# melspectrum007/audio-visual-speech-enhancement

Hardware: NVIDIA B200
Metric: audio-sec/sec (higher is better)
Workload: dtype f32

## Files before the change

audio-visual-speech-enhancement_b200/csrc/avse_fwd4_stages.cuh:

```cuda
#pragma once
#include "avse_common.h"
#include "avse_dft.cuh"
#include "avse_fwd_stages.cuh"

#if !defined(AVSE_DB_FAST_MINMAX)
#define AVSE_DB_FAST_MINMAX 0
#endif
#if !defined(AVSE_SCAN4_UNROLL)
#define AVSE_SCAN4_UNROLL 8
#endif

namespace avse {

constexpr int F4 = 4;
constexpr int CHUNK4 = 41;
constexpr int SCAN4_BINS = 8 * CHUNK4;
constexpr int FRAME4_F = N1 * ROW_F + 16;
constexpr int ZERO4_F = N1 * ROW_F;
#ifndef AVSE_SCAN4_BLK
#define AVSE_SCAN4_BLK 4
#endif
#ifndef AVSE_DB_BRANCHFREE_EXTRA
#define AVSE_DB_BRANCHFREE_EXTRA 1
#endif
constexpr int FLUSH4_F = 1284;
constexpr int WARP4_SMEM_F = F4 * FRAME4_F;
constexpr int RAW4 = 16 + 4 * (F4 - 1);
static_assert(FLUSH4_F + 48 <= FRAME4_F && (FLUSH4_F % 2) == 0, "flush area");

struct Lane4Const {
    float win[16];
    vec2 tw[16];
};

AVSE_HD void lane4_const_init(int lane, const float* s_win, const vec2* s_tw, Lane4Const& lc) {
#pragma unroll
    for (int j = 0; j < 16; ++j) { lc.win[j] = s_win[N2 * j + lane]; lc.tw[j] = s_tw[j * N2 + lane]; }
}

template <typename S, bool TILED>
AVSE_HD bool group4_interior(const FwdTileT<S>& tl, int& nz_shift) {
    nz_shift = 0;
    const int a = tl.t0 * HOP - HALF;
    if (!(tl.nz != nullptr && a >= 0 && (tl.t0 + 3) * HOP + HALF <= tl.vmin && tl.t0 + 3 < tl.T)) return false;
    if (TILED && tl.period_n > 0) {
        const int j = a + tl.phase_n;
        const int q = j / tl.period_n;
        if ((j + (F4 - 1) * HOP + NFFT - 1) / tl.period_n != q) return false;
        nz_shift = tl.phase_n - q * tl.period_n;
    }
    return true;
}

AVSE_HD void p4_column(cpx (&x)[16], const vec2 (&tw)[16], float* dst) {
    dft16(x);
    cstore(dst, x[0]);
#pragma unroll
    for (int k1 = 1; k1 < 16; ++k1) cstore(dst + k1 * ROW_F, cmul(x[k1], tw[k1].x, tw[k1].y));
}

template <typename S>
AVSE_HD void p4_load_raw(const FwdTileT<S>& tl, int nz_shift, int lane, float (&rs)[RAW4], float (&rn)[RAW4]) {
    const int o = tl.t0 * HOP - HALF + lane;
    const S* ps = tl.sp + o;
    const S* pn = tl.nz + (o + nz_shift);
#pragma unroll
    for (int j = 0; j < RAW4; ++j) { rs[j] = (float)ps[N2 * j]; rn[j] = (float)pn[N2 * j]; }
}

#if !defined(AVSE_F4_REFLECT_FAST)
#define AVSE_F4_REFLECT_FAST 1
#endif
AVSE_HD int reflect_index(int i, int L) {
    i = i < 0 ? -i : i;
    const int m = 2 * (L - 1) - i;
    return i < m ? i : m;
}

template <typename S, bool PAD>
AVSE_HD bool group4_reflect_only(const FwdTileT<S>& tl) {
    return tl.nz != nullptr && (PAD || tl.vmin >= tl.L) && tl.period_n == 0 && tl.L >= 4 * NFFT;
}

template <typename S, bool PAD>
AVSE_HD void p4_load_raw_reflect(const FwdTileT<S>& tl, int lane, float (&rs)[RAW4], float (&rn)[RAW4]) {
    const int o = tl.t0 * HOP - HALF + lane;
    if (!PAD || tl.vmin >= tl.L) {
#pragma unroll
        for (int j = 0; j < RAW4; ++j) { const int i = reflect_index(o + N2 * j, tl.L); rs[j] = (float)tl.sp[i]; rn[j] = (float)tl.nz[i]; }
    } else {
#pragma unroll
        for (int j = 0; j < RAW4; ++j) {
            const int i = reflect_index(o + N2 * j, tl.L);
            rs[j] = i < tl.valid_s ? (float)tl.sp[i] : 0.0f;
            rn[j] = i < tl.valid_n ? (float)tl.nz[i] : 0.0f;
        }
    }
}

template <typename S, bool PAD>
AVSE_HD void p4_load_tail_raw_reflect(const FwdTileT<S>& tl, int lane, float (&rs)[16], float (&rn)[16]) {
    const int o = (tl.t0 + (lane >> 3)) * HOP - HALF + 32 + (lane & 7);
    if (!PAD || tl.vmin >= tl.L) {
#pragma unroll
        for (int j = 0; j < 16; ++j) { const int i = reflect_index(o + N2 * j, tl.L); rs[j] = (float)tl.sp[i]; rn[j] = (float)tl.nz[i]; }
    } else {
#pragma unroll
        for (int j = 0; j < 16; ++j) {
            const int i = reflect_index(o + N2 * j, tl.L);
            rs[j] = i < tl.valid_s ? (float)tl.sp[i] : 0.0f;
            rn[j] = i < tl.valid_n ? (float)tl.nz[i] : 0.0f;
        }
    }
}

template <typename S>
AVSE_HD void stage4_store_pcm_guarded(const FwdTileT<S>& tl, int lane, const float (&rs)[RAW4], const float (&rn)[RAW4], const float (&ts)[16],
                                      const float (&tn)[16]) {
    if (tl.mixed_pcm == nullptr) return;
    const int i0 = tl.t0 * HOP + lane;
#pragma unroll
    for (int j = 8; j < 24; ++j) {
        const int i = i0 + N2 * (j - 8);
        if (i < tl.L) tl.mixed_pcm[i] = rs[j] + tl.factor * (rn[j] * tl.gain);
    }
    const int i1 = (tl.t0 + (lane >> 3)) * HOP + 32 + (lane & 7);
#pragma unroll
    for (int j = 0; j < 4; ++j) {
        const int i = i1 + N2 * j;
        if (i < tl.L) tl.mixed_pcm[i] = ts[8 + j] + tl.factor * (tn[8 + j] * tl.gain);
    }
}

#if !defined(AVSE_P1_ROLL)
#define AVSE_P1_ROLL 9
#endif
template <typename S>
AVSE_HD void stage4_pass1_main(const FwdTileT<S>& tl, int lane, float (&rs)[RAW4], float (&rn)[RAW4],
                               const Lane4Const& lc, float* frames) {
    const float gain = tl.gain;
#if AVSE_P1_ROLL == 9
#pragma unroll
    for (int j = 0; j < RAW4; ++j) rn[j] *= gain;
    if (tl.mixed_pcm != nullptr) {
        float* pm = tl.mixed_pcm + tl.t0 * HOP + lane;
#pragma unroll
        for (int j = 8; j < 24; ++j) pm[N2 * (j - 8)] = rs[j] + tl.factor * rn[j];
    }
#pragma unroll
    for (int f = 0; f < F4; ++f) {
        cpx x[16];
#pragma unroll
        for (int j = 0; j < 16; ++j) x[j] = cmake(rs[4 * f + j] * lc.win[j], rn[4 * f + j] * lc.win[j]);
        p4_column(x, lc.tw, frames + f * FRAME4_F + 2 * lane);
    }
#elif AVSE_P1_ROLL == 0
#pragma unroll
    for (int j = 0; j < 12; ++j) rn[j] *= gain;
#pragma unroll
    for (int f = 0; f < F4; ++f) {
#pragma unroll
        for (int j = 12; j < 16; ++j) rn[4 * f + j] *= gain;
        if (tl.mixed_pcm != nullptr) {
            float* pm = tl.mixed_pcm + (tl.t0 + f) * HOP + lane;
#pragma unroll
            for (int j = 0; j < 4; ++j) pm[N2 * j] = rs[4 * f + 8 + j] + tl.factor * rn[4 * f + 8 + j];
        }
        cpx x[16];
#pragma unroll
        for (int j = 0; j < 16; ++j) x[j] = cmake(rs[4 * f + j] * lc.win[j], rn[4 * f + j] * lc.win[j]);
        p4_column(x, lc.tw, frames + f * FRAME4_F + 2 * lane);
    }
#else
    constexpr int STEP = AVSE_P1_ROLL == 4 ? 1 : 2;
    constexpr int W = 16 + 4 * (STEP - 1);
#pragma unroll
    for (int j = 0; j < 12; ++j) rn[j] *= gain;
    float* pm = tl.mixed_pcm != nullptr ? tl.mixed_pcm + tl.t0 * HOP + lane : nullptr;
    float* dst = frames + 2 * lane;
#pragma unroll 1
    for (int it = 0; it < F4 / STEP; ++it) {
#pragma unroll
        for (int j = 12; j < W; ++j) rn[j] *= gain;
#pragma unroll
        for (int f = 0; f < STEP; ++f) {
            if (pm != nullptr) {
#pragma unroll
                for (int j = 0; j < 4; ++j) pm[N2 * j] = rs[4 * f + 8 + j] + tl.factor * rn[4 * f + 8 + j];
                pm += HOP;
            }
            cpx x[16];
#pragma unroll
            for (int j = 0; j < 16; ++j) x[j] = cmake(rs[4 * f + j] * lc.win[j], rn[4 * f + j] * lc.win[j]);
            p4_column(x, lc.tw, dst);
            dst += FRAME4_F;
        }
#pragma unroll
        for (int j = 0; j + 4 * STEP < RAW4; ++j) { rs[j] = rs[j + 4 * STEP]; rn[j] = rn[j + 4 * STEP]; }
    }
#endif
}

template <typename S>
AVSE_HD void p4_load_tail_raw(const FwdTileT<S>& tl, int nz_shift, int lane, float (&rs)[16], float (&rn)[16]) {
    const int f = lane >> 3, n2 = 32 + (lane & 7);
    const int o = (tl.t0 + f) * HOP - HALF + n2;
    const S* ps = tl.sp + o;
    const S* pn = tl.nz + (o + nz_shift);
#pragma unroll
    for (int j = 0; j < 16; ++j) { rs[j] = (float)ps[N2 * j]; rn[j] = (float)pn[N2 * j]; }
}

template <typename S>
AVSE_HD void stage4_pass1_tail_compute(const FwdTileT<S>& tl, int lane, const float (&rs)[16], float (&rn)[16], const float* s_win,
                                       const vec2* s_tw, float* frames) {
    const int f = lane >> 3, n2 = 32 + (lane & 7);
#pragma unroll
    for (int j = 0; j < 16; ++j) rn[j] *= tl.gain;
    vec2 tw[16];
#pragma unroll
    for (int k1 = 1; k1 < 16; ++k1) tw[k1] = s_tw[k1 * N2 + n2];
    tw[0].x = 1.0f; tw[0].y = 0.0f;
    if (tl.mixed_pcm != nullptr) {
        float* pm = tl.mixed_pcm + (tl.t0 + f) * HOP + n2;
#pragma unroll
        for (int j = 0; j < 4; ++j) pm[N2 * j] = rs[8 + j] + tl.factor * rn[8 + j];
    }
    cpx x[16];
#pragma unroll
    for (int j = 0; j < 16; ++j) { const float w = s_win[N2 * j + n2]; x[j] = cmake(rs[j] * w, rn[j] * w); }
    p4_column(x, tw, frames + f * FRAME4_F + 2 * n2);
}

template <typename S>
AVSE_HD void stage4_pass1_tail(const FwdTileT<S>& tl, int nz_shift, int lane, const float* s_win, const vec2* s_tw, float* frames) {
    float rs[16], rn[16];
    p4_load_tail_raw(tl, nz_shift, lane, rs, rn);
    stage4_pass1_tail_compute(tl, lane, rs, rn, s_win, s_tw, frames);
}

template <typename S>
AVSE_HD void stage4_pass1_unified(const FwdTileT<S>& tl, int lane, float (&rs)[RAW4], float (&rn)[RAW4], const float (&ts)[16], float (&tn)[16],
                                  const Lane4Const& lc, const float* s_win, const vec2* s_tw, float* frames) {
    const float gain = tl.gain;
    const int tf = lane >> 3, tn2 = 32 + (lane & 7);
#pragma unroll
    for (int j = 0; j < RAW4; ++j) rn[j] *= gain;
#pragma unroll
    for (int j = 0; j < 16; ++j) tn[j] *= gain;
    if (tl.mixed_pcm != nullptr) {
        float* pm = tl.mixed_pcm + tl.t0 * HOP + lane;
#pragma unroll
        for (int j = 8; j < 24; ++j) pm[N2 * (j - 8)] = rs[j] + tl.factor * rn[j];
        float* pt = tl.mixed_pcm + (tl.t0 + tf) * HOP + tn2;
#pragma unroll
        for (int j = 0; j < 4; ++j) pt[N2 * j] = ts[8 + j] + tl.factor * tn[8 + j];
    }
    vec2 tw[16];
    tw[0].x = 1.0f; tw[0].y = 0.0f;
#pragma unroll 1
    for (int round = 0; round < 5; ++round) {
        if (round == 0 || round == 4) {
            const int n2 = round == 0 ? lane : tn2;
#pragma unroll
            for (int k1 = 1; k1 < 16; ++k1) tw[k1] = s_tw[k1 * N2 + n2];
        }
        cpx x[16];
        float* dst;
        switch (round) {
        case 0:
#pragma unroll
            for (int j = 0; j < 16; ++j) x[j] = cmake(rs[j] * lc.win[j], rn[j] * lc.win[j]);
            dst = frames + 2 * lane;
            break;
        case 1:
#pragma unroll
            for (int j = 0; j < 16; ++j) x[j] = cmake(rs[4 + j] * lc.win[j], rn[4 + j] * lc.win[j]);
            dst = frames + FRAME4_F + 2 * lane;
            break;
        case 2:
#pragma unroll
            for (int j = 0; j < 16; ++j) x[j] = cmake(rs[8 + j] * lc.win[j], rn[8 + j] * lc.win[j]);
            dst = frames + 2 * FRAME4_F + 2 * lane;
            break;
        case 3:
#pragma unroll
            for (int j = 0; j < 16; ++j) x[j] = cmake(rs[12 + j] * lc.win[j], rn[12 + j] * lc.win[j]);
            dst = frames + 3 * FRAME4_F + 2 * lane;
            break;
        default:
#pragma unroll
            for (int j = 0; j < 16; ++j) { const float w = s_win[N2 * j + tn2]; x[j] = cmake(ts[j] * w, tn[j] * w); }
            dst = frames + tf * FRAME4_F + 2 * tn2;
            break;
        }
        p4_column(x, tw, dst);
    }
}

template <typename S, bool TILED>
AVSE_HD void stage4_pass1_edge(const FwdTileT<S>& tl, int lane, const float* s_win, const vec2* s_tw, float* frames) {
#pragma unroll 1
    for (int round = 0; round < 5; ++round) {
        const int f = round < 4 ? round : lane >> 3;
        const int n2 = round < 4 ? lane : 32 + (lane & 7);
        const int t_raw = tl.t0 + f;
        const int t = t_raw < tl.T ? t_raw : tl.T - 1;
        const int base = t * HOP - HALF + n2;
        float rs[16], rn[16];
#pragma unroll
        for (int j = 0; j < 16; ++j) {
            rs[j] = load_sample_edge(tl.sp, base + N2 * j, tl.L, tl.valid_s);
            rn[j] = tl.gain * load_sample_edge(tl.nz, base + N2 * j, tl.L, tl.valid_n, TILED ? tl.period_n : 0, TILED ? tl.phase_n : 0);
        }
        if (tl.mixed_pcm != nullptr && t_raw < tl.T) {
#pragma unroll
            for (int j = 0; j < 4; ++j) {
                const int i = t * HOP + N2 * j + n2;
                if (i < tl.L) tl.mixed_pcm[i] = rs[8 + j] + tl.factor * rn[8 + j];
            }
        }
        vec2 tw[16];
#pragma unroll
        for (int k1 = 1; k1 < 16; ++k1) tw[k1] = s_tw[k1 * N2 + n2];
        tw[0].x = 1.0f; tw[0].y = 0.0f;
        cpx x[16];
#pragma unroll
        for (int j = 0; j < 16; ++j) { const float w = s_win[N2 * j + n2]; x[j] = cmake(rs[j] * w, rn[j] * w); }
        p4_column(x, tw, frames + f * FRAME4_F + 2 * n2);
    }
}

AVSE_HD void p4_pass2_load(int lane, int r, const float* frames, cpx (&x)[40]) {
    const int f = 2 * r + (lane >> 4), k1 = lane & 15;
    const float* row = frames + f * FRAME4_F + k1 * ROW_F;
#pragma unroll
    for (int q = 0; q < 20; ++q) cload2(row + 4 * q, x[2 * q], x[2 * q + 1]);
}

AVSE_HD void p4_pass2_compute(int lane, int r, const float* frames, cpx (&x)[40]) {
    p4_pass2_load(lane, r, frames, x);
    dft40_inplace(x);
}

AVSE_HD void p4_pass2_store(int lane, int r, float* frames, const cpx (&x)[40]) {
    const int f = 2 * r + (lane >> 4), k1 = lane & 15;
    float* z = frames + f * FRAME4_F + 2 * k1;
#pragma unroll
    for (int c = 0; c < 5; ++c)
#pragma unroll
        for (int d = 0; d < 8; ++d) {
            const int idx = (8 * c + 5 * d) % 40;
            const int k2 = (16 * c + 25 * d) % 40;
            cstore(z + 2 * N1 * k2, x[idx]);
        }
}

AVSE_HD float fma_rn(float a, float b, float c) { return fmaf(a, b, c); }

AVSE_HD void scan4_bin(const float* za, const float* zc, const vec2* tab, int j, bool emit, float factor, float nfactor,
                       float*& esn, float*& em, cpx& Asn, cpx& Bsn, float& Am, float& Bm) {
    const cpx a = cload(za + 2 * j);
    const cpx c = cload(zc - 2 * j);
    const vec2 w = tab[j];
    if (emit) {
        cstore(esn, Asn);
        *em = Am;
        esn += 2;
        em -= 1;
        Asn = Bsn; Am = Bm;
        Bsn = cmake(0.0f, 0.0f); Bm = 0.0f;
    }
    const cpx s = cfma_pp(c, cmake(1.0f, -1.0f), a);
    const cpx n = cfma_pp(c, cmake(-1.0f, 1.0f), a);
    const float mr = fma_rn(factor, cim(n), cre(s));
    const float mi = fma_rn(nfactor, cre(n), cim(s));
    const float ms = fast_sqrt(fma_rn(cim(s), cim(s), cre(s) * cre(s)));
    const float mn = fast_sqrt(fma_rn(cim(n), cim(n), cre(n) * cre(n)));
    const float mm = fast_sqrt(fma_rn(mi, mi, mr * mr));
    const cpx msn = cmake(ms, mn);
    Asn = cfma_pp(msn, cmake(w.x, w.x), Asn);
    Bsn = cfma_pp(msn, cmake(w.y, w.y), Bsn);
    Am = fma_rn(w.x, mm, Am);
    Bm = fma_rn(w.y, mm, Bm);
}

AVSE_HD void stage4_scan(int lane, float factor, const vec2* s_w, unsigned mask_lo, unsigned mask_hi, float* frames) {
    const int f = lane >> 3, p = lane & 7;
    float* fr = frames + f * FRAME4_F;
    const float* za = fr + 2 * CHUNK4 * p;
    const float* zc = fr + 2 * (NFFT - CHUNK4 * p);
    const vec2* tab = s_w + CHUNK4 * p;
    float* esn = fr + 2 * CHUNK4 * p;
    float* em = fr + 2 * (NFFT - CHUNK4 * p) + 1;
    cpx Asn = cmake(0.0f, 0.0f), Bsn = cmake(0.0f, 0.0f);
    float Am = 0.0f, Bm = 0.0f;
    const float nfactor = -factor;
    unsigned mlo = mask_lo, mhi = mask_hi;
    static_assert(CHUNK4 == 41 && (40 % AVSE_SCAN4_BLK) == 0 && AVSE_SCAN4_BLK < 32, "blocks of AVSE_SCAN4_BLK bins + 1");
#pragma unroll 1
    for (int ib = 0; ib < 40; ib += AVSE_SCAN4_BLK) {
#pragma unroll
        for (int j = 0; j < AVSE_SCAN4_BLK; ++j) scan4_bin(za, zc, tab, j, ((mlo >> j) & 1u) != 0u, factor, nfactor, esn, em, Asn, Bsn, Am, Bm);
        za += 2 * AVSE_SCAN4_BLK; zc -= 2 * AVSE_SCAN4_BLK; tab += AVSE_SCAN4_BLK;
        mlo = (mlo >> AVSE_SCAN4_BLK) | (mhi << (32 - AVSE_SCAN4_BLK));
        mhi >>= AVSE_SCAN4_BLK;
    }
    scan4_bin(za, zc, tab, 0, (mlo & 1u) != 0u, factor, nfactor, esn, em, Asn, Bsn, Am, Bm);
    float* fl = fr + FLUSH4_F + 6 * p;
    cstore(fl + 0, Asn);
    cstore(fl + 2, Bsn);
    cstore(fl + 4, cmake(Am, Bm));
}

AVSE_HD void stage4_db(int lane, int q, float factor, const ivec4* s_loc, const float* frames, const FwdOut& out, int t0, int T,
                       float (&mx)[3], float* mn) {
    const int m = 32 * q + lane;
    if (m >= NMEL) return;
    const ivec4 loc = s_loc[m];
    float mel[3][F4];
#pragma unroll
    for (int f = 0; f < F4; ++f) {
        const float* fr = frames + f * FRAME4_F;
        const vec2 sn = *reinterpret_cast<const vec2*>(fr + (loc.x & 0xffff));
        mel[0][f] = sn.x; mel[1][f] = sn.y; mel[2][f] = fr[loc.x >> 16];
    }
#if AVSE_DB_BRANCHFREE_EXTRA
    {
#pragma unroll
        for (int f = 0; f < F4; ++f) {
            const float* fr = frames + f * FRAME4_F;
            const vec2 sn = *reinterpret_cast<const vec2*>(fr + (loc.y & 0xffff));
            mel[0][f] += sn.x; mel[1][f] += sn.y; mel[2][f] += fr[loc.y >> 16];
        }
    }
#else
    if ((loc.y & 0xffff) != ZERO4_F) {
#pragma unroll
        for (int f = 0; f < F4; ++f) {
            const float* fr = frames + f * FRAME4_F;
            const vec2 sn = *reinterpret_cast<const vec2*>(fr + (loc.y & 0xffff));
            mel[0][f] += sn.x; mel[1][f] += sn.y; mel[2][f] += fr[loc.y >> 16];
        }
    }
#endif
    if (loc.z >= 0) {
#pragma unroll
        for (int f = 0; f < F4; ++f) {
            const float* fr = frames + f * FRAME4_F;
            const vec2 sn = *reinterpret_cast<const vec2*>(fr + (loc.z & 0xffff));
            mel[0][f] += sn.x; mel[1][f] += sn.y; mel[2][f] += fr[loc.z >> 16];
        }
    }
    const int nvalid = T - t0 < F4 ? T - t0 : F4;
    int off;
    bool store = true;
    if (out.layout == 0) {
        const int sl = t0 / SPSS, tt = t0 - sl * SPSS;
        off = (sl * NMEL + m) * SPSS + tt;
        store = sl < out.n_slices;
    } else {
        off = m * out.ld_t + t0;
    }
#pragma unroll
    for (int sig = 0; sig < 3; ++sig) {
        const float scale = sig == 1 ? factor : 1.0f;
        float d[F4];
        float lm = neg_inf(), ln = -neg_inf();
#pragma unroll
        for (int f = 0; f < F4; ++f) d[f] = amp_to_db(mel[sig][f] * scale);
#if AVSE_DB_FAST_MINMAX
        if (nvalid == F4) {
            lm = fmaxf(fmaxf(d[0], d[1]), fmaxf(d[2], d[3]));
            ln = fminf(fminf(d[0], d[1]), fminf(d[2], d[3]));
        } else
#endif
        {
#pragma unroll
            for (int f = 0; f < F4; ++f) {
                const bool v = f < nvalid;
                lm = v ? fmaxf(lm, d[f]) : lm;
                ln = v ? fminf(ln, d[f]) : ln;
            }
        }
        mx[sig] = fmaxf(lm, mx[sig]);
        float* dst = out.dst[sig];
        mn[32 * sig + lane] = fminf(mn[32 * sig + lane], (dst != nullptr && store) ? ln : -neg_inf());
        if (dst != nullptr && store) {
            if (out.layout == 0) {
                vec4 o; o.x = d[0]; o.y = d[1]; o.z = d[2]; o.w = d[3];
                *reinterpret_cast<vec4*>(dst + off) = o;
            } else {
#pragma unroll
                for (int f = 0; f < F4; ++f)
                    if (f < nvalid) dst[off + f] = d[f];
            }
        }
    }
}

#if !defined(AVSE_DB_SPLIT_LAST)
#define AVSE_DB_SPLIT_LAST 1
#endif
AVSE_HD void stage4_db_last(int lane, float factor, const ivec4* s_loc, const float* frames, const FwdOut& out, int t0, int T,
                            float (&mx)[3], float* mn) {
    const int half = lane >> 4, m = 64 + (lane & 15), f0 = 2 * half;
    const ivec4 loc = s_loc[m];
    float mel[3][2];
#pragma unroll
    for (int f = 0; f < 2; ++f) {
        const float* fr = frames + (f0 + f) * FRAME4_F;
        const vec2 sn = *reinterpret_cast<const vec2*>(fr + (loc.x & 0xffff));
        mel[0][f] = sn.x; mel[1][f] = sn.y; mel[2][f] = fr[loc.x >> 16];
        const vec2 s2 = *reinterpret_cast<const vec2*>(fr + (loc.y & 0xffff));
        mel[0][f] += s2.x; mel[1][f] += s2.y; mel[2][f] += fr[loc.y >> 16];
    }
    if (loc.z >= 0) {
#pragma unroll
        for (int f = 0; f < 2; ++f) {
            const float* fr = frames + (f0 + f) * FRAME4_F;
            const vec2 sn = *reinterpret_cast<const vec2*>(fr + (loc.z & 0xffff));
            mel[0][f] += sn.x; mel[1][f] += sn.y; mel[2][f] += fr[loc.z >> 16];
        }
    }
    const int nvalid = T - t0 < F4 ? T - t0 : F4;
    int off;
    bool store = true;
    if (out.layout == 0) {
        const int sl = t0 / SPSS, tt = t0 - sl * SPSS;
        off = (sl * NMEL + m) * SPSS + tt + f0;
        store = sl < out.n_slices;
    } else {
        off = m * out.ld_t + t0 + f0;
    }
#pragma unroll
    for (int sig = 0; sig < 3; ++sig) {
        const float scale = sig == 1 ? factor : 1.0f;
        float d[2];
        float lm = neg_inf(), ln = -neg_inf();
#pragma unroll
        for (int f = 0; f < 2; ++f) {
            d[f] = amp_to_db(mel[sig][f] * scale);
            const bool v = f0 + f < nvalid;
            lm = v ? fmaxf(lm, d[f]) : lm;
            ln = v ? fminf(ln, d[f]) : ln;
        }
        mx[sig] = fmaxf(lm, mx[sig]);
        float* dst = out.dst[sig];
        mn[32 * sig + lane] = fminf(mn[32 * sig + lane], (dst != nullptr && store) ? ln : -neg_inf());
        if (dst != nullptr && store) {
            if (out.layout == 0) {
                vec2 o; o.x = d[0]; o.y = d[1];
                *reinterpret_cast<vec2*>(dst + off) = o;
            } else {
#pragma unroll
                for (int f = 0; f < 2; ++f)
                    if (f0 + f < nvalid) dst[off + f] = d[f];
            }
        }
    }
}

}
```

audio-visual-speech-enhancement_b200/csrc/avse_kernels.cu:

```cuda
#include <cuda_runtime.h>
#include <cooperative_groups.h>
#include <cstdio>
#include <cstring>
#include <cstdlib>
#include <string>
#include <vector>
#include <new>

#include "../../include/avse_b200.h"
#include "avse_common.h"
#include "avse_tables.h"
#include "avse_ctx.h"
#include "avse_fwd_stages.cuh"
#include "avse_fwd4_stages.cuh"

using namespace avse;

static thread_local std::string g_err;
int avse_fail(int code, const std::string& msg) { g_err = msg; return code; }
int avse_cuda_fail(cudaError_t e, const char* where) {
    g_err = std::string(where) + ": " + cudaGetErrorString(e);
    return (int)e;
}

// ... 634 lines not shown
#pragma unroll
        for (int s = 0; s < 3; ++s) {
            float v = mx[s], w = mn[32 * s + lane];
#pragma unroll
            for (int o = 16; o > 0; o >>= 1) {
                v = fmaxf(v, __shfl_xor_sync(0xffffffffu, v, o));
                w = fminf(w, __shfl_xor_sync(0xffffffffu, w, o));
            }
            if (lane == 0) {
                atomicMax(A.max_key + 3 * uu + s, float_to_key(v));
                if (A.min_key) atomicMin(A.min_key + 3 * uu + s, float_to_key(w));
            }
            mx[s] = neg_inf();
            mn[32 * s + lane] = -neg_inf();
        }
    };

    auto prefetch_ahead = [&](int it, int u, int g, const FwdTileT<S>& tc) {
#if AVSE_F4_PREFETCH > 0
        if (it + AVSE_F4_PREFETCH < n_tiles) {
            int g2 = g + AVSE_F4_PREFETCH, u2 = u;
            if (g2 >= P.G) { g2 -= P.G; ++u2; }
            const int lo = g2 == 0 ? 0 : g2 * (F4 * HOP) + HOP;
            const int hi = g2 * (F4 * HOP) + (NFFT + HOP);
            const int i0 = (lo & ~(LINE - 1)) + LINE * lane;
            if (TILED) {
                if (u2 == u && i0 < hi && i0 < tc.valid_s && lane < 22) {
                    asm volatile("prefetch.global.L2 [%0];" ::"l"(tc.sp + i0));
                    if (tc.period_n == 0 && i0 < tc.valid_n) asm volatile("prefetch.global.L2 [%0];" ::"l"(tc.nz + i0));
                }
            } else if (i0 < hi && i0 < A.L && i0 < A.in_stride && lane < 22) {
                const size_t o = (size_t)u2 * A.in_stride + i0;
                asm volatile("prefetch.global.L2 [%0];" ::"l"(in_speech + o));
                asm volatile("prefetch.global.L2 [%0];" ::"l"(in_noise + o));
            }
        }
#endif
    };
    auto load_utt = [&](int uu, int& ovs, int& ovn, float& of) {
        ovs = A.len_speech ? A.len_speech[uu] : A.L;
        ovn = A.len_noise ? A.len_noise[uu] : ovs;
        ovs = ovs < 0 ? 0 : (ovs < A.L ? ovs : A.L);
        ovn = ovn < 0 ? 0 : (ovn < A.L ? ovn : A.L);
        const MixGain mg = mix_gain(A, uu);
        of = mg.resid;
        utt_sm[UF * (uu & 1)] = mg.gain;
#if AVSE_F4_PTR_SLOT
        {
            float** ps = reinterpret_cast<float**>(utt_sm + UF * (uu & 1) + 2);
            ps[0] = A.out_speech ? A.out_speech + (size_t)uu * A.out_stride : nullptr;
            ps[1] = A.out_noise ? A.out_noise + (size_t)uu * A.out_stride : nullptr;
            ps[2] = A.out_mixed ? A.out_mixed + (size_t)uu * A.out_stride : nullptr;
            ps[3] = A.mixed_pcm ? A.mixed_pcm + (size_t)uu * A.pcm_stride : nullptr;
        }
#endif
        if (TILED) {
            const S* sp;
            const S* nz;
            int period, phase;
            if (P.pool.speech_index != nullptr) {
                const PoolRow r = pool_row(P.pool, uu);
                ovs = r.ls < A.L ? r.ls : A.L;
                ovn = ovs;
                sp = in_speech + r.s_off;
                nz = in_noise + r.n_off;
                period = r.ln;
                phase = r.off;
            } else {
                sp = in_speech + (size_t)uu * A.in_stride;
                nz = in_noise + (size_t)uu * A.in_stride;
                period = A.noise_period[uu];
                phase = 0;
            }
            fit_noise_row(nz, period, phase, ovn);
            int* si = reinterpret_cast<int*>(utt_sm + UF * (uu & 1));
            si[1] = period;
            si[F4_UTT_F + 4] = phase;
            const S** pi = reinterpret_cast<const S**>(utt_sm + UF * (uu & 1) + F4_UTT_F);
            pi[0] = sp;
            pi[1] = nz;
        }
    };
    auto make_tile = [&](int uu, int gg, int tvs, int tvn, float tf) {
        FwdTileT<S> t;
        if (TILED) {
            const S* const* pi = reinterpret_cast<const S* const*>(utt_sm + UF * (uu & 1) + F4_UTT_F);
            t.sp = pi[0];
            t.nz = pi[1];
        } else {
            t.sp = in_speech + (size_t)uu * A.in_stride;
            t.nz = in_noise + (size_t)uu * A.in_stride;
        }
        t.L = A.L;
        t.valid_s = tvs;
        t.valid_n = tvn;
        t.vmin = tvs < tvn ? tvs : tvn;
        t.T = P.T;
        t.t0 = gg * F4;
        t.factor = tf;
        t.gain = 0.0f;
        t.period_n = TILED ? reinterpret_cast<const int*>(utt_sm)[UF * (uu & 1) + 1] : 0;
        t.phase_n = TILED ? reinterpret_cast<const int*>(utt_sm)[UF * (uu & 1) + F4_UTT_F + 4] : 0;
#if AVSE_F4_PTR_SLOT
        t.mixed_pcm = reinterpret_cast<float* const*>(utt_sm + UF * (uu & 1) + 2)[3];
#else
        t.mixed_pcm = A.mixed_pcm ? A.mixed_pcm + (size_t)uu * A.pcm_stride : nullptr;
#endif
        return t;
    };
    load_utt(u, vs, vn, factor);
    FwdTileT<S> tl = make_tile(u, g, vs, vn, factor);
    int nz_shift = 0;
    bool interior = group4_interior<S, TILED>(tl, nz_shift);
    bool reflect = AVSE_F4_REFLECT_FAST && !TILED && !interior && group4_reflect_only<S, PAD>(tl);
    float rs[RAW4], rn[RAW4], ts[16], tn[16];
    if (interior) {
        p4_load_raw(tl, nz_shift, lane, rs, rn);
        p4_load_tail_raw(tl, nz_shift, lane, ts, tn);
    } else if (reflect) {
        p4_load_raw_reflect<S, PAD>(tl, lane, rs, rn);
        p4_load_tail_raw_reflect<S, PAD>(tl, lane, ts, tn);
    }
#pragma unroll 1
    for (int it = 0; it < n_tiles; ++it) {
        prefetch_ahead(it, u, g, tl);
        tl.gain = utt_sm[UF * (u & 1)];
        if (reflect) {
            stage4_store_pcm_guarded(tl, lane, rs, rn, ts, tn);
            tl.mixed_pcm = nullptr;
        }
        if (interior || reflect) {
#if AVSE_P1_UNIFIED
            stage4_pass1_unified(tl, lane, rs, rn, ts, tn, lc, s_win, s_tw, frames);
#else
            stage4_pass1_main(tl, lane, rs, rn, lc, frames);
            stage4_pass1_tail_compute(tl, lane, ts, tn, s_win, s_tw, frames);
#endif
        } else {
            stage4_pass1_edge<S, TILED>(tl, lane, s_win, s_tw, frames);
        }
        __syncwarp();

#pragma unroll 1
        for (int r = 0; r < 2; ++r) {
            cpx x[40];
            p4_pass2_compute(lane, r, frames, x);
            __syncwarp();
            p4_pass2_store(lane, r, frames, x);
        }
        __syncwarp();

        stage4_scan(lane, tl.factor, s_scanw, mask_lo, mask_hi, frames);
        __syncwarp();

        int u2 = u, g2 = g + 1;
        int vs2 = vs, vn2 = vn;
        float factor2 = tl.factor;
        const bool last_of_utt = g2 == P.G;
        const bool have_next = it + 1 < n_tiles;
        if (last_of_utt) { g2 = 0; ++u2; if (have_next) load_utt(u2, vs2, vn2, factor2); }
        FwdTileT<S> tnx = make_tile(have_next ? u2 : u, have_next ? g2 : g, vs2, vn2, factor2);
        int nz_shift2 = 0;
        const bool interior2 = have_next && group4_interior<S, TILED>(tnx, nz_shift2);
        const bool reflect2 = AVSE_F4_REFLECT_FAST && !TILED && have_next && !interior2 && group4_reflect_only<S, PAD>(tnx);
        if (interior2) {
            p4_load_raw(tnx, nz_shift2, lane, rs, rn);
            p4_load_tail_raw(tnx, nz_shift2, lane, ts, tn);
        } else if (reflect2) {
            p4_load_raw_reflect<S, PAD>(tnx, lane, rs, rn);
            p4_load_tail_raw_reflect<S, PAD>(tnx, lane, ts, tn);
        }

        {
            FwdOut out;
#if AVSE_F4_PTR_SLOT
            float* const* ps = reinterpret_cast<float* const*>(utt_sm + UF * (u & 1) + 2);
            out.dst[0] = ps[0]; out.dst[1] = ps[1]; out.dst[2] = ps[2];
#else
            out.dst[0] = A.out_speech ? A.out_speech + (size_t)u * A.out_stride : nullptr;
            out.dst[1] = A.out_noise ? A.out_noise + (size_t)u * A.out_stride : nullptr;
            out.dst[2] = A.out_mixed ? A.out_mixed + (size_t)u * A.out_stride : nullptr;
#endif
            out.layout = A.layout;
            out.n_slices = A.n_slices;
            out.ld_t = A.ld_t;
#pragma unroll 1
#if AVSE_DB_SPLIT_LAST && AVSE_DB_BRANCHFREE_EXTRA
            for (int q = 0; q < 2; ++q) stage4_db(lane, q, tl.factor, s_loc, frames, out, g * F4, P.T, mx, mn);
            stage4_db_last(lane, tl.factor, s_loc, frames, out, g * F4, P.T, mx, mn);
#else
            for (int q = 0; q < 3; ++q) stage4_db(lane, q, tl.factor, s_loc, frames, out, g * F4, P.T, mx, mn);
#endif
        }
        __syncwarp();

        if (last_of_utt || !have_next) flush_max(u);
        u = u2; g = g2; vs = vs2; vn = vn2;
        tl = tnx;
        interior = interior2;
        reflect = reflect2;
    }
}

__global__ void avse_reset_max_kernel(int* __restrict__ max_key, int* __restrict__ min_key, int n, int min_value);

static int forward_launch(avse_ctx* ctx, const avse_forward_args& a, const PoolRows& pool, void* stream) {
    if (a.B <= 0 || a.L <= HALF) return avse_fail(AVSE_E_ARG, "avse_forward: need B > 0 and L > 320 (reflect padding)");
    if (a.layout != AVSE_LAYOUT_SLICES && a.layout != AVSE_LAYOUT_SPEC) return avse_fail(AVSE_E_ARG, "avse_forward: bad layout");
    FwdParams P;
    P.a = a;
    P.pool = pool;
    P.tb = ctx->fwd;
    P.T = 1 + a.L / HOP;
    P.G = (P.T + FPG - 1) / FPG;
    if (a.layout == AVSE_LAYOUT_SLICES) {
        if (a.n_slices < 0 || (long long)a.n_slices * AVSE_SPSS > P.T) return avse_fail(AVSE_E_ARG, "avse_forward: n_slices exceeds int(T/20) (dp:50)");
        if (a.out_stride < (long long)a.n_slices * NMEL * AVSE_SPSS) return avse_fail(AVSE_E_ARG, "avse_forward: out_stride too small");
    } else {
        if (a.ld_t < P.T) return avse_fail(AVSE_E_ARG, "avse_forward: ld_t < T");
        if (a.out_stride < (long long)NMEL * a.ld_t) return avse_fail(AVSE_E_ARG, "avse_forward: out_stride too small");
    }
    if (a.mixed_pcm && a.pcm_stride < a.L) return avse_fail(AVSE_E_ARG, "avse_forward: pcm_stride < L");
    float* outs[3] = {a.out_speech, a.out_noise, a.out_mixed};
    for (int s = 0; s < 3; ++s)
        if (outs[s] && (((size_t)outs[s] & 15) || (a.out_stride & 3))) return avse_fail(AVSE_E_ARG, "avse_forward: outputs must be 16-byte aligned with out_stride % 4 == 0");
    const long long total = (long long)a.B * P.G;
    if (total > 0x7fffffffLL) return avse_fail(AVSE_E_ARG, "avse_forward: B * groups exceeds 2^31; split the batch");

    static thread_local int configured_dev = -1;
    int dev = 0;
    CUDA_TRY(cudaGetDevice(&dev));
    if (dev != ctx->device) return avse_fail(AVSE_E_ARG, "avse_forward: current device differs from the context's device");
    if (a.sample_format != AVSE_SAMPLE_F32 && a.sample_format != AVSE_SAMPLE_I16) return avse_fail(AVSE_E_ARG, "avse_forward: bad sample_format");
    const bool i16 = a.sample_format == AVSE_SAMPLE_I16;
    const bool use_f4 = ctx->f4_tables && a.noise != nullptr && a.stft_speech == nullptr && (!ctx->force_f2 || i16);
    if (i16 && !use_f4) return avse_fail(AVSE_E_ARG, "avse_forward: int16 samples are supported for pair batches (noise != NULL, no stft_speech) with the standard 2-tap filterbank; convert to float32 first");
    if (use_f4) {
        static thread_local int configured4_dev = -1;
        if (configured4_dev != dev) {
            CUDA_TRY(cudaFuncSetAttribute(avse_forward4_kernel<float, false, false>, cudaFuncAttributeMaxDynamicSharedMemorySize, F4_SMEM_BYTES));
            CUDA_TRY(cudaFuncSetAttribute(avse_forward4_kernel<short, false, false>, cudaFuncAttributeMaxDynamicSharedMemorySize, F4_SMEM_BYTES));
            CUDA_TRY(cudaFuncSetAttribute(avse_forward4_kernel<float, false, true>, cudaFuncAttributeMaxDynamicSharedMemorySize, F4_SMEM_BYTES));
            CUDA_TRY(cudaFuncSetAttribute(avse_forward4_kernel<short, false, true>, cudaFuncAttributeMaxDynamicSharedMemorySize, F4_SMEM_BYTES));
            CUDA_TRY(cudaFuncSetAttribute(avse_forward4_kernel<float, true, false>, cudaFuncAttributeMaxDynamicSharedMemorySize, F4_SMEM_BYTES));
            CUDA_TRY(cudaFuncSetAttribute(avse_forward4_kernel<short, true, false>, cudaFuncAttributeMaxDynamicSharedMemorySize, F4_SMEM_BYTES));
            configured4_dev = dev;
        }
        P.G = (P.T + F4 - 1) / F4;
        const long long total4 = (long long)a.B * P.G;
        long long blocks4 = ctx->num_sms;
        const long long need4 = (total4 + F4_WARPS - 1) / F4_WARPS;
        if (blocks4 > need4) blocks4 = need4;
        const long long nwarps4 = blocks4 * F4_WARPS;
        P.total_tiles = (int)total4;
        P.per_warp = (int)((total4 + nwarps4 - 1) / nwarps4);
        P.split = make_warp_split(total4, blocks4, F4_WARPS);
        const bool tiled = a.noise_period != nullptr || pool.speech_index != nullptr;
        const bool pad = !tiled && (a.len_speech != nullptr || a.len_noise != nullptr);
        const cudaStream_t st4 = (cudaStream_t)stream;
        if (i16 && tiled) avse_forward4_kernel<short, true, false><<<(unsigned)blocks4, F4_THREADS, F4_SMEM_BYTES, st4>>>(P);
        else if (tiled) avse_forward4_kernel<float, true, false><<<(unsigned)blocks4, F4_THREADS, F4_SMEM_BYTES, st4>>>(P);
        else if (i16 && pad) avse_forward4_kernel<short, false, true><<<(unsigned)blocks4, F4_THREADS, F4_SMEM_BYTES, st4>>>(P);
        else if (pad) avse_forward4_kernel<float, false, true><<<(unsigned)blocks4, F4_THREADS, F4_SMEM_BYTES, st4>>>(P);
        else if (i16) avse_forward4_kernel<short, false, false><<<(unsigned)blocks4, F4_THREADS, F4_SMEM_BYTES, st4>>>(P);
        else avse_forward4_kernel<float, false, false><<<(unsigned)blocks4, F4_THREADS, F4_SMEM_BYTES, st4>>>(P);
        CUDA_TRY(cudaGetLastError());
        return 0;
    }
    if (configured_dev != dev) {
        CUDA_TRY(cudaFuncSetAttribute(avse_forward_kernel<true>, cudaFuncAttributeMaxDynamicSharedMemorySize, FWD_SMEM_BYTES));
        CUDA_TRY(cudaFuncSetAttribute(avse_forward_kernel<false>, cudaFuncAttributeMaxDynamicSharedMemorySize, FWD_SMEM_BYTES));
        configured_dev = dev;
    }
    long long blocks = (long long)FWD_CTAS * ctx->num_sms;
    const long long need = (total + FWD_WARPS - 1) / FWD_WARPS;
    if (blocks > need) blocks = need;
    const long long nwarps = blocks * FWD_WARPS;
    P.total_tiles = (int)total;
    P.per_warp = (int)((total + nwarps - 1) / nwarps);
    if (ctx->std_tables) avse_forward_kernel<true><<<(unsigned)blocks, FWD_THREADS, FWD_SMEM_BYTES, (cudaStream_t)stream>>>(P);
    else avse_forward_kernel<false><<<(unsigned)blocks, FWD_THREADS, FWD_SMEM_BYTES, (cudaStream_t)stream>>>(P);
    CUDA_TRY(cudaGetLastError());
    if (a.min_key) {
        avse_reset_max_kernel<<<(3 * a.B + 255) / 256, 256, 0, (cudaStream_t)stream>>>(nullptr, a.min_key, 3 * a.B, (int)0x80000000);
        CUDA_TRY(cudaGetLastError());
    }
    return 0;
}

extern "C" int avse_forward(avse_ctx* ctx, const avse_forward_args* args, void* stream) {
    if (!ctx || !args) return avse_fail(AVSE_E_ARG, "avse_forward: NULL argument");
    if (ctx->generic) return avse_generic_forward(ctx, args, nullptr, stream);
    const avse_forward_args& a = *args;
    if (!a.speech || !a.max_key) return avse_fail(AVSE_E_ARG, "avse_forward: speech and max_key are required");
    if (a.B <= 0 || a.L <= HALF) return avse_fail(AVSE_E_ARG, "avse_forward: need B > 0 and L > 320 (reflect padding)");
    if (!a.len_speech && a.in_stride < a.L) return avse_fail(AVSE_E_ARG, "avse_forward: in_stride < L needs len_speech");
    const PoolRows identity = {};
    return forward_launch(ctx, a, identity, stream);
}

#ifndef AVSE_FLOOR_ZLOOP
#define AVSE_FLOOR_ZLOOP 1
#endif
static __device__ __forceinline__ void floor_store(float4* q, float4 v, float thr) {
    if (fminf(fminf(v.x, v.y), fminf(v.z, v.w)) < thr) {
        v.x = fmaxf(v.x, thr); v.y = fmaxf(v.y, thr); v.z = fmaxf(v.z, thr); v.w = fmaxf(v.w, thr);
        *q = v;
    }
}

__global__ void __launch_bounds__(256) avse_floor_inplace_kernel(float* __restrict__ data0, float* __restrict__ data1,
                                                                 float* __restrict__ data2, long long stride, long long n_per_utt,
                                                                 const int* __restrict__ max_key, const int* __restrict__ min_key,
                                                                 int which0, int n_sig) {
    const int u = blockIdx.x;
#if AVSE_FLOOR_ZLOOP
    for (int z = 0; z < n_sig; ++z) {
#else
    const int z = blockIdx.z;
    {
#endif
    float* data = z == 0 ? data0 : (z == 1 ? data1 : data2);
    const float thr = key_to_float(max_key[3 * u + which0 + z]) - TOP_DB;
#if AVSE_FLOOR_ZLOOP
    if (min_key != nullptr && key_to_float(min_key[3 * u + which0 + z]) >= thr) continue;
#else
    if (min_key != nullptr && key_to_float(min_key[3 * u + which0 + z]) >= thr) return;
#endif
    float* p = data + (size_t)u * stride;
    const long long n4 = n_per_utt >> 2;
    const long long step = (long long)gridDim.y * blockDim.x;
    long long i = (long long)blockIdx.y * blockDim.x + threadIdx.x;
    for (; i + 3 * step < n4; i += 4 * step) {
        float4* q = reinterpret_cast<float4*>(p) + i;
        const float4 v0 = q[0], v1 = q[step], v2 = q[2 * step], v3 = q[3 * step];
        floor_store(q, v0, thr);
        floor_store(q + step, v1, thr);
        floor_store(q + 2 * step, v2, thr);
        floor_store(q + 3 * step, v3, thr);
    }
    for (; i < n4; i += step) {
        float4 v = reinterpret_cast<float4*>(p)[i];
        if (fminf(fminf(v.x, v.y), fminf(v.z, v.w)) < thr) {
            v.x = fmaxf(v.x, thr); v.y = fmaxf(v.y, thr); v.z = fmaxf(v.z, thr); v.w = fmaxf(v.w, thr);
            reinterpret_cast<float4*>(p)[i] = v;
        }
    }
    for (long long j = 4 * n4 + (long long)blockIdx.y * blockDim.x + threadIdx.x; j < n_per_utt; j += step)
        p[j] = fmaxf(p[j], thr);
    }
}

static unsigned floor_grid_x(long long n_per_utt) {
    long long bx = (n_per_utt / 4 + 256 * 8 - 1) / (256 * 8);
    if (bx < 1) bx = 1;
    if (bx > 256) bx = 256;
    return (unsigned)bx;
}

extern "C" int avse_floor_inplace3(avse_ctx* ctx, float* speech, float* noise, float* mixed, long long stride, long long n_per_utt,
                                   int B, const int* max_key, const int* min_key, void* stream) {
    if (!ctx || !speech || !noise || !mixed || !max_key) return avse_fail(AVSE_E_ARG, "avse_floor_inplace3: NULL argument");
    if (B <= 0 || n_per_utt <= 0 || stride < n_per_utt) return avse_fail(AVSE_E_ARG, "avse_floor_inplace3: bad sizes");
    if ((((size_t)speech | (size_t)noise | (size_t)mixed) & 15) || (stride & 3))
        return avse_fail(AVSE_E_ARG, "avse_floor_inplace3: data must be 16-byte aligned with stride % 4 == 0");
    dim3 grid((unsigned)B, floor_grid_x(n_per_utt), AVSE_FLOOR_ZLOOP ? 1 : 3);
    avse_floor_inplace_kernel<<<grid, 256, 0, (cudaStream_t)stream>>>(speech, noise, mixed, stride, n_per_utt, max_key, min_key, 0, 3);
    CUDA_TRY(cudaGetLastError());
    return 0;
}

extern "C" int avse_floor_inplace(avse_ctx* ctx, float* data, long long stride, long long n_per_utt, int B, const int* max_key,
                                  const int* min_key, int which, void* stream) {
    if (!ctx || !data || !max_key) return avse_fail(AVSE_E_ARG, "avse_floor_inplace: NULL argument");
    if (B <= 0 || n_per_utt <= 0 || stride < n_per_utt || which < 0 || which > 2) return avse_fail(AVSE_E_ARG, "avse_floor_inplace: bad sizes");
    if (((size_t)data & 15) || (stride & 3)) return avse_fail(AVSE_E_ARG, "avse_floor_inplace: data must be 16-byte aligned with stride % 4 == 0");
    dim3 grid((unsigned)B, floor_grid_x(n_per_utt));
    avse_floor_inplace_kernel<<<grid, 256, 0, (cudaStream_t)stream>>>(data, data, data, stride, n_per_utt, max_key, min_key, which, 1);
    CUDA_TRY(cudaGetLastError());
    return 0;
}

__global__ void __launch_bounds__(256) avse_floor_gather_kernel(const float* __restrict__ spec, long long spec_stride, int ld_t,
                                                                float* __restrict__ slices, long long slices_stride, int n_slices,
                                                                const int* __restrict__ max_key, int which, int n_mels, int spss) {
    const int u = blockIdx.x;
    const float thr = key_to_float(max_key[3 * u + which]) - TOP_DB;
    const float* src = spec + (size_t)u * spec_stride;
    float* dst = slices + (size_t)u * slices_stride;
    const int n = n_slices * n_mels * spss;
    for (int i = blockIdx.y * blockDim.x + threadIdx.x; i < n; i += gridDim.y * blockDim.x) {
        const int j = i % spss;
        const int m = (i / spss) % n_mels;
        const int s = i / (spss * n_mels);
        dst[i] = fmaxf(src[(size_t)m * ld_t + s * spss + j], thr);
    }
}

extern "C" int avse_floor_gather(avse_ctx* ctx, const float* spec, long long spec_stride, int ld_t, float* slices,
                                 long long slices_stride, int n_slices, int B, const int* max_key, int which, void* stream) {
    if (!ctx || !spec || !slices || !max_key) return avse_fail(AVSE_E_ARG, "avse_floor_gather: NULL argument");
    if (B <= 0 || n_slices <= 0 || ld_t < n_slices * ctx->spss || which < 0 || which > 2) return avse_fail(AVSE_E_ARG, "avse_floor_gather: bad sizes");
    const int n = n_slices * ctx->n_mels * ctx->spss;
    int bx = (n + 255) / 256;
    if (bx > 64) bx = 64;
    dim3 grid((unsigned)B, (unsigned)bx);
    avse_floor_gather_kernel<<<grid, 256, 0, (cudaStream_t)stream>>>(spec, spec_stride, ld_t, slices, slices_stride, n_slices, max_key, which,
                                                                     ctx->n_mels, ctx->spss);
    CUDA_TRY(cudaGetLastError());
    return 0;
}

__global__ void avse_reset_max_kernel(int* __restrict__ max_key, int* __restrict__ min_key, int n, int min_value) {
    const int i = blockIdx.x * blockDim.x + threadIdx.x;
    if (i < n) {
        if (max_key) max_key[i] = (int)0x80000000;
        if (min_key) min_key[i] = min_value;
    }
}

extern "C" int avse_reset_max(avse_ctx* ctx, int* max_key, int* min_key, int n, void* stream) {
    if (!ctx || !max_key || n <= 0) return avse_fail(AVSE_E_ARG, "avse_reset_max: bad argument");
    avse_reset_max_kernel<<<(n + 255) / 256, 256, 0, (cudaStream_t)stream>>>(max_key, min_key, n, 0x7fffffff);
    CUDA_TRY(cudaGetLastError());
    return 0;
}

__global__ void avse_max_db_kernel(const int* __restrict__ max_key, int n, float* __restrict__ out) {
    const int i = blockIdx.x * blockDim.x + threadIdx.x;
    if (i < n) out[i] = key_to_float(max_key[i]);
}

extern "C" int avse_max_db(avse_ctx* ctx, const int* max_key, int n, float* out_db, void* stream) {
    if (!ctx || !max_key || !out_db || n <= 0) return avse_fail(AVSE_E_ARG, "avse_max_db: bad argument");
    avse_max_db_kernel<<<(n + 255) / 256, 256, 0, (cudaStream_t)stream>>>(max_key, n, out_db);
    CUDA_TRY(cudaGetLastError());
    return 0;
}

extern "C" int avse_mix_pooled(avse_ctx* ctx, const avse_pool_mix_args* args, void* stream) {
    if (!ctx || !args) return avse_fail(AVSE_E_ARG, "avse_mix_pooled: NULL argument");
    const avse_pool_mix_args& m = *args;
    if (!m.speech_pool || !m.noise_pool || !m.speech_len || !m.noise_len || !m.speech_index || !m.noise_index)
        return avse_fail(AVSE_E_ARG, "avse_mix_pooled: pools, clip lengths and row indices are required");
    if (!m.out_speech || !m.out_noise || !m.out_mixed || !m.factor_out || !m.max_key || !m.bad_row_flag)
        return avse_fail(AVSE_E_ARG, "avse_mix_pooled: the three slice outputs, factor_out, max_key and bad_row_flag are required");
    if (m.n_speech <= 0 || m.n_noise <= 0 || m.speech_stride <= 0 || m.noise_stride <= 0)
        return avse_fail(AVSE_E_ARG, "avse_mix_pooled: empty pool (n_speech, n_noise and both strides must be > 0)");
    if (m.B <= 0 || m.n_slices <= 0) return avse_fail(AVSE_E_ARG, "avse_mix_pooled: need B > 0 and n_slices > 0");
    if (m.sample_format != AVSE_SAMPLE_F32 && m.sample_format != AVSE_SAMPLE_I16) return avse_fail(AVSE_E_ARG, "avse_mix_pooled: bad sample_format");
    PoolRows pool;
    pool.speech_index = m.speech_index;
    pool.noise_index = m.noise_index;
    pool.noise_offset = m.noise_offset;
    pool.speech_len = m.speech_len;
    pool.noise_len = m.noise_len;
    pool.speech_stride = m.speech_stride;
    pool.noise_stride = m.noise_stride;
    pool.n_speech = m.n_speech;
    pool.n_noise = m.n_noise;
    pool.bad_row_flag = m.bad_row_flag;
    avse_forward_args a = {};
    a.speech = m.speech_pool;
    a.noise = m.noise_pool;
    a.factor = m.factor_out;
    a.B = m.B;
    a.L = m.L;
    a.layout = AVSE_LAYOUT_SLICES;
    a.n_slices = m.n_slices;
    a.out_speech = m.out_speech;
    a.out_noise = m.out_noise;
    a.out_mixed = m.out_mixed;
    a.out_stride = m.out_stride;
    a.mixed_pcm = m.mixed_pcm;
    a.pcm_stride = m.pcm_stride;
    a.max_key = m.max_key;
    a.min_key = m.min_key;
    a.sample_format = m.sample_format;
    a.equalizer = m.equalizer_out;
    const int half = ctx->generic ? ctx->n_fft / 2 : HALF;
    if (m.L <= half) return avse_fail(AVSE_E_ARG, "avse_mix_pooled: need L > n_fft / 2 (reflect padding)");
    const int T = ctx->generic ? avse_generic_frames(ctx->gen.geo, m.L) : 1 + m.L / HOP;
    if ((long long)m.n_slices * ctx->spss > T) return avse_fail(AVSE_E_ARG, "avse_mix_pooled: n_slices exceeds int(T / spss) (dp:50)");
    const long long n_per_utt = (long long)m.n_slices * ctx->n_mels * ctx->spss;
    if (m.out_stride < n_per_utt) return avse_fail(AVSE_E_ARG, "avse_mix_pooled: out_stride too small");
    float* outs[3] = {m.out_speech, m.out_noise, m.out_mixed};
    for (int s = 0; s < 3; ++s)
        if (((size_t)outs[s] & 15) || (m.out_stride & 3)) return avse_fail(AVSE_E_ARG, "avse_mix_pooled: outputs must be 16-byte aligned with out_stride % 4 == 0");
    if (m.mixed_pcm && m.pcm_stride < m.L) return avse_fail(AVSE_E_ARG, "avse_mix_pooled: pcm_stride < L");
    if (m.sample_format == AVSE_SAMPLE_I16 && !ctx->generic && !ctx->f4_tables)
        return avse_fail(AVSE_E_ARG, "avse_mix_pooled: int16 samples need the standard 2-tap filterbank; convert the pools to float32 first");
    int dev = 0;
    CUDA_TRY(cudaGetDevice(&dev));
    if (dev != ctx->device) return avse_fail(AVSE_E_ARG, "avse_mix_pooled: current device differs from the context's device");

    const int longest = m.speech_stride < 0x7fffffffLL ? (int)m.speech_stride : 0x7fffffff;
    int rc = snr_factor_launch(ctx, m.speech_pool, m.noise_pool, m.sample_format, 0, nullptr, nullptr, m.B, longest, pool, m.snr_db,
                               m.factor_out, m.equalizer_out, m.max_key, m.min_key, stream);
    if (rc != 0) return rc;
    rc = ctx->generic ? avse_generic_forward(ctx, &a, &pool, stream) : forward_launch(ctx, a, pool, stream);
    if (rc != 0) return rc;
    return avse_floor_inplace3(ctx, m.out_speech, m.out_noise, m.out_mixed, m.out_stride, n_per_utt, m.B, m.max_key, m.min_key, stream);
}

__global__ void __launch_bounds__(256) avse_gather_rows_kernel(const float* __restrict__ s0, const float* __restrict__ s1,
                                                               const float* __restrict__ s2, long long src_rows,
                                                               const long long* __restrict__ index, long long n_out, int row4,
                                                               float* __restrict__ d0, float* __restrict__ d1, float* __restrict__ d2,
                                                               int* __restrict__ bad) {
    const int z = blockIdx.y;
    const float4* src = reinterpret_cast<const float4*>(z == 0 ? s0 : (z == 1 ? s1 : s2));
    float4* dst = reinterpret_cast<float4*>(z == 0 ? d0 : (z == 1 ? d1 : d2));
    const int lane = threadIdx.x & 31;
    const long long warp = ((long long)blockIdx.x * blockDim.x + threadIdx.x) >> 5;
    const long long nwarps = ((long long)gridDim.x * blockDim.x) >> 5;
    for (long long i = warp; i < n_out; i += nwarps) {
        const long long r = index[i];
        if (r < 0 || r >= src_rows) { if (lane == 0) atomicExch(bad, 1); continue; }
        const float4* sp = src + r * row4;
        float4* dp = dst + i * row4;
        int j = lane;
        for (; j + 96 < row4; j += 128) {
            const float4 a = sp[j], b = sp[j + 32], c = sp[j + 64], d = sp[j + 96];
            dp[j] = a; dp[j + 32] = b; dp[j + 64] = c; dp[j + 96] = d;
        }
        for (; j < row4; j += 32) dp[j] = sp[j];
    }
}

extern "C" int avse_gather_rows(avse_ctx* ctx, const float* src0, const float* src1, const float* src2, long long src_rows,
                                long long row_elems, const long long* index, long long n_out, float* dst0, float* dst1, float* dst2,
                                int* bad_index_flag, void* stream) {
    if (!ctx || !src0 || !dst0 || !index) return avse_fail(AVSE_E_ARG, "avse_gather_rows: NULL argument");
    if ((src1 == nullptr) != (dst1 == nullptr) || (src2 == nullptr) != (dst2 == nullptr) || (src2 && !src1))
        return avse_fail(AVSE_E_ARG, "avse_gather_rows: src/dst arrays must be given in matching pairs, in order");
    if (src_rows <= 0 || n_out <= 0 || row_elems <= 0 || (row_elems & 3) || row_elems > 0x7fffffffLL * 4)
        return avse_fail(AVSE_E_ARG, "avse_gather_rows: row_elems must be a positive multiple of 4");
    const float* ps[6] = {src0, src1, src2, dst0, dst1, dst2};
    for (int i = 0; i < 6; ++i)
        if ((size_t)ps[i] & 15) return avse_fail(AVSE_E_ARG, "avse_gather_rows: arrays must be 16-byte aligned");
    if (!bad_index_flag) return avse_fail(AVSE_E_ARG, "avse_gather_rows: bad_index_flag (device int, zeroed by the caller) is required");
    const int narr = src2 ? 3 : (src1 ? 2 : 1);
    long long bx = (n_out + 7) / 8;
    const long long cap = (long long)ctx->num_sms * 16;
    if (bx > cap) bx = cap;
    dim3 grid((unsigned)bx, (unsigned)narr);
    avse_gather_rows_kernel<<<grid, 256, 0, (cudaStream_t)stream>>>(src0, src1, src2, src_rows, index, n_out, (int)(row_elems / 4),
                                                                    dst0, dst1, dst2, bad_index_flag);
    CUDA_TRY(cudaGetLastError());
    return 0;
}
```

Measured before the change: 4.740 million.

## Add L2 eviction hints for dB stores and rework floor kernel unrolling

Speech-channel dB outputs are now stored with an L2 evict_last cache policy, so the later in-place floor pass is more likely to hit in L2. An optional streaming-store path for the other outputs and the mixed PCM is added but off by default. The floor kernel's main loop becomes a bounds-guarded unroll over four elements with no separate remainder loop. The grid sizing divisor drops from 256*8 to 256*4, which roughly doubles the number of floor blocks. Pinning speech data in L2 may push other data out of the cache.

```diff
diff --git a/audio-visual-speech-enhancement_b200/csrc/avse_fwd4_stages.cuh b/audio-visual-speech-enhancement_b200/csrc/avse_fwd4_stages.cuh
--- a/audio-visual-speech-enhancement_b200/csrc/avse_fwd4_stages.cuh
+++ b/audio-visual-speech-enhancement_b200/csrc/avse_fwd4_stages.cuh
@@ -32,6 +32,20 @@
     float win[16];
     vec2 tw[16];
 };
+
+#ifndef AVSE_F4_KEEP_SPEECH
+#define AVSE_F4_KEEP_SPEECH 1
+#endif
+#ifndef AVSE_F4_STREAM_REST
+#define AVSE_F4_STREAM_REST 0
+#endif
+AVSE_HD void pcm_store(float* p, float v) {
+#if defined(__CUDA_ARCH__) && AVSE_F4_STREAM_REST
+    asm volatile("st.global.cs.f32 [%0], %1;" :: "l"(p), "f"(v) : "memory");
+#else
+    *p = v;
+#endif
+}
 
 AVSE_HD void lane4_const_init(int lane, const float* s_win, const vec2* s_tw, Lane4Const& lc) {
 #pragma unroll
@@ -145,7 +159,7 @@
     if (tl.mixed_pcm != nullptr) {
         float* pm = tl.mixed_pcm + tl.t0 * HOP + lane;
 #pragma unroll
-        for (int j = 8; j < 24; ++j) pm[N2 * (j - 8)] = rs[j] + tl.factor * rn[j];
+        for (int j = 8; j < 24; ++j) pcm_store(pm + N2 * (j - 8), rs[j] + tl.factor * rn[j]);
     }
 #pragma unroll
     for (int f = 0; f < F4; ++f) {
@@ -224,7 +238,7 @@
     if (tl.mixed_pcm != nullptr) {
         float* pm = tl.mixed_pcm + (tl.t0 + f) * HOP + n2;
 #pragma unroll
-        for (int j = 0; j < 4; ++j) pm[N2 * j] = rs[8 + j] + tl.factor * rn[8 + j];
+        for (int j = 0; j < 4; ++j) pcm_store(pm + N2 * j, rs[8 + j] + tl.factor * rn[8 + j]);
     }
     cpx x[16];
 #pragma unroll
@@ -413,6 +427,43 @@
     cstore(fl + 4, cmake(Am, Bm));
 }
 
+template <int SIG>
+AVSE_HD void db_store4(float* p, const vec4& o) {
+#if defined(__CUDA_ARCH__) && AVSE_F4_KEEP_SPEECH
+    if (SIG == 0) {
+        asm volatile("{\n\t.reg .b64 pol;\n\tcreatepolicy.fractional.L2::evict_last.b64 pol, 1.0;\n\t"
+                     "st.global.L2::cache_hint.v4.f32 [%0], {%1, %2, %3, %4}, pol;\n\t}"
+                     :: "l"(p), "f"(o.x), "f"(o.y), "f"(o.z), "f"(o.w) : "memory");
+        return;
+    }
+#endif
+#if defined(__CUDA_ARCH__) && AVSE_F4_STREAM_REST
+    if (SIG != 0) {
+        asm volatile("st.global.cs.v4.f32 [%0], {%1, %2, %3, %4};" :: "l"(p), "f"(o.x), "f"(o.y), "f"(o.z), "f"(o.w) : "memory");
+        return;
+    }
+#endif
+    *reinterpret_cast<vec4*>(p) = o;
+}
+template <int SIG>
+AVSE_HD void db_store2(float* p, const vec2& o) {
+#if defined(__CUDA_ARCH__) && AVSE_F4_KEEP_SPEECH
+    if (SIG == 0) {
+        asm volatile("{\n\t.reg .b64 pol;\n\tcreatepolicy.fractional.L2::evict_last.b64 pol, 1.0;\n\t"
+                     "st.global.L2::cache_hint.v2.f32 [%0], {%1, %2}, pol;\n\t}"
+                     :: "l"(p), "f"(o.x), "f"(o.y) : "memory");
+        return;
+    }
+#endif
+#if defined(__CUDA_ARCH__) && AVSE_F4_STREAM_REST
+    if (SIG != 0) {
+        asm volatile("st.global.cs.v2.f32 [%0], {%1, %2};" :: "l"(p), "f"(o.x), "f"(o.y) : "memory");
+        return;
+    }
+#endif
+    *reinterpret_cast<vec2*>(p) = o;
+}
+
 AVSE_HD void stage4_db(int lane, int q, float factor, const ivec4* s_loc, const float* frames, const FwdOut& out, int t0, int T,
                        float (&mx)[3], float* mn) {
     const int m = 32 * q + lane;
@@ -489,7 +540,7 @@
         if (dst != nullptr && store) {
             if (out.layout == 0) {
                 vec4 o; o.x = d[0]; o.y = d[1]; o.z = d[2]; o.w = d[3];
-                *reinterpret_cast<vec4*>(dst + off) = o;
+                if (sig == 0) db_store4<0>(dst + off, o); else db_store4<1>(dst + off, o);
             } else {
 #pragma unroll
                 for (int f = 0; f < F4; ++f)
@@ -551,7 +602,7 @@
         if (dst != nullptr && store) {
             if (out.layout == 0) {
                 vec2 o; o.x = d[0]; o.y = d[1];
-                *reinterpret_cast<vec2*>(dst + off) = o;
+                if (sig == 0) db_store2<0>(dst + off, o); else db_store2<1>(dst + off, o);
             } else {
 #pragma unroll
                 for (int f = 0; f < 2; ++f)
diff --git a/audio-visual-speech-enhancement_b200/csrc/avse_kernels.cu b/audio-visual-speech-enhancement_b200/csrc/avse_kernels.cu
--- a/audio-visual-speech-enhancement_b200/csrc/avse_kernels.cu
+++ b/audio-visual-speech-enhancement_b200/csrc/avse_kernels.cu
@@ -960,6 +960,7 @@
 #ifndef AVSE_FLOOR_ZLOOP
 #define AVSE_FLOOR_ZLOOP 1
 #endif
+constexpr int FLOOR_K = 4;
 static __device__ __forceinline__ void floor_store(float4* q, float4 v, float thr) {
     if (fminf(fminf(v.x, v.y), fminf(v.z, v.w)) < thr) {
         v.x = fmaxf(v.x, thr); v.y = fmaxf(v.y, thr); v.z = fmaxf(v.z, thr); v.w = fmaxf(v.w, thr);
@@ -989,20 +990,15 @@
     const long long n4 = n_per_utt >> 2;
     const long long step = (long long)gridDim.y * blockDim.x;
     long long i = (long long)blockIdx.y * blockDim.x + threadIdx.x;
-    for (; i + 3 * step < n4; i += 4 * step) {
+    for (; i < n4; i += FLOOR_K * step) {
         float4* q = reinterpret_cast<float4*>(p) + i;
-        const float4 v0 = q[0], v1 = q[step], v2 = q[2 * step], v3 = q[3 * step];
-        floor_store(q, v0, thr);
-        floor_store(q + step, v1, thr);
-        floor_store(q + 2 * step, v2, thr);
-        floor_store(q + 3 * step, v3, thr);
-    }
-    for (; i < n4; i += step) {
-        float4 v = reinterpret_cast<float4*>(p)[i];
-        if (fminf(fminf(v.x, v.y), fminf(v.z, v.w)) < thr) {
-            v.x = fmaxf(v.x, thr); v.y = fmaxf(v.y, thr); v.z = fmaxf(v.z, thr); v.w = fmaxf(v.w, thr);
-            reinterpret_cast<float4*>(p)[i] = v;
-        }
+        float4 v[FLOOR_K];
+#pragma unroll
+        for (int k = 0; k < FLOOR_K; ++k)
+            if (i + k * step < n4) v[k] = q[k * step];
+#pragma unroll
+        for (int k = 0; k < FLOOR_K; ++k)
+            if (i + k * step < n4) floor_store(q + k * step, v[k], thr);
     }
     for (long long j = 4 * n4 + (long long)blockIdx.y * blockDim.x + threadIdx.x; j < n_per_utt; j += step)
         p[j] = fmaxf(p[j], thr);
@@ -1010,7 +1006,7 @@
 }
 
 static unsigned floor_grid_x(long long n_per_utt) {
-    long long bx = (n_per_utt / 4 + 256 * 8 - 1) / (256 * 8);
+    long long bx = (n_per_utt / 4 + 256 * FLOOR_K - 1) / (256 * FLOOR_K);
     if (bx < 1) bx = 1;
     if (bx > 256) bx = 256;
     return (unsigned)bx;
```

Result: faster. 4.789 million, median of 6 (+1.0%).
